# biomedia-mira/causal-gen

Hardware: AMD Instinct MI355X
Metric: HVAE train images/sec (higher is better)
Workload: dtype f16; 1 GPU; ukbb192 HVAE train step (192x192x1, DGauss likelihood, beta=5.0, z_max_res=96); per_gpu_batch=32, global_batch=32, parallelism=dp1, hipgraph=True, params=17371122

## Files before the change

causal-gen_amd/_lib.py:

```python
import ctypes as C
import os

_HERE = os.path.dirname(os.path.abspath(__file__))
LIB_PATH = os.environ.get("CGEN_LIB") or os.path.join(_HERE, "libcgen_hip.so")

F32, F16, F32S = 0, 1, 2
DMOL_LOW_BIT = 0x100
ACT_NONE, ACT_RELU, ACT_GELU = 0, 1, 2
UNARY_LEAKY_RELU, UNARY_CLAMP_MIN, UNARY_ADD = 3, 4, 5
MAX_SEG = 4


class View(C.Structure):
    _fields_ = [("p", C.c_void_p), ("sn", C.c_int64), ("sh", C.c_int64), ("sw", C.c_int64), ("c", C.c_int32),
                ("cpad", C.c_int32)]


NULL_VIEW = View(None, 0, 0, 0, 0, 0)


class ConvArgs(C.Structure):
    _fields_ = [("dtype", C.c_int32), ("n", C.c_int32), ("h", C.c_int32), ("w", C.c_int32), ("ks", C.c_int32),
                ("nseg", C.c_int32), ("act", C.c_int32), ("dact", C.c_int32), ("seg", View * MAX_SEG),
                ("weight", C.c_void_p), ("bias", C.c_void_p), ("out", View), ("aux", View), ("res1", View), ("res2", View),
                ("out_rem", C.c_int64), ("res1_rem", C.c_int64)]


class Block3Out(C.Structure):
    _fields_ = [("w", C.c_void_p), ("bias", C.c_void_p), ("out", View), ("aux", View), ("res1", View),
                ("out_rem", C.c_int64), ("res1_rem", C.c_int64)]


class Block3Args(C.Structure):
    _fields_ = [("dtype", C.c_int32), ("n", C.c_int32), ("h", C.c_int32), ("w", C.c_int32), ("nseg", C.c_int32),
                ("nout", C.c_int32), ("pre_act", C.c_int32), ("reserved", C.c_int32), ("seg", View * MAX_SEG),
                ("w_a", C.c_void_p), ("bias_a", C.c_void_p), ("mid", View), ("mid_aux", View), ("o", Block3Out * 2), ("w_a16", C.c_void_p)]


class Block4Args(C.Structure):
    _fields_ = [("dtype", C.c_int32), ("n", C.c_int32), ("h", C.c_int32), ("w", C.c_int32), ("nseg", C.c_int32),
                ("nout", C.c_int32), ("fwd", C.c_int32), ("b", C.c_int32), ("seg", View * MAX_SEG),
                ("wimg", C.c_void_p * 3), ("bias", C.c_void_p * 3), ("mid", View * 3), ("mid_aux", View * 3), ("o", Block3Out * 3)]


class WgradArgs(C.Structure):
    _fields_ = [("dtype", C.c_int32), ("n", C.c_int32), ("h", C.c_int32), ("w", C.c_int32), ("ks", C.c_int32),
                ("nseg", C.c_int32), ("act", C.c_int32), ("nsplit", C.c_int32), ("seg", View * MAX_SEG), ("gout", View),
                ("partial_w", C.c_void_p), ("partial_b", C.c_void_p)]


class WprepDesc(C.Structure):
    _fields_ = [("src", C.c_void_p), ("dst", C.c_void_p), ("co", C.c_int32), ("ci_total", C.c_int32), ("ks", C.c_int32),
                ("mode", C.c_int32), ("nseg", C.c_int32), ("seg_off", C.c_int32), ("seg_c", C.c_int32 * MAX_SEG),
                ("dtype", C.c_int32), ("rows_pad", C.c_int32), ("k_pad", C.c_int32), ("reserved", C.c_int32),
                ("numel", C.c_int64)]


class WredDesc(C.Structure):
    _fields_ = [("partial_w", C.c_void_p), ("partial_b", C.c_void_p), ("grad_w", C.c_void_p), ("grad_b", C.c_void_p),
                ("co", C.c_int32), ("ci_total", C.c_int32), ("ks", C.c_int32), ("nsplit", C.c_int32),
                ("accumulate", C.c_int32), ("unscale", C.c_float), ("layout", C.c_int32), ("reserved", C.c_int32),
                ("numel", C.c_int64)]


class AdamwArgs(C.Structure):
    _fields_ = [("p", C.c_void_p), ("g", C.c_void_p), ("m", C.c_void_p), ("v", C.c_void_p), ("ema", C.c_void_p),
                ("count", C.c_int64), ("lr", C.c_float), ("beta1", C.c_float), ("beta2", C.c_float), ("eps", C.c_float),
                ("wd", C.c_float), ("ema_beta", C.c_float), ("warmup_steps", C.c_int32), ("ema_update_after", C.c_int32),
                ("state_dev", C.c_void_p)]


class PredHead(C.Structure):
    _fields_ = [("c", C.c_int32), ("res", C.c_int32), ("width", C.c_int32), ("nout", C.c_int32), ("ctx", C.c_int32),
                ("kind", C.c_int32), ("tanh_loc", C.c_int32), ("obs_stride", C.c_int32), ("std_fixed", C.c_float),
                ("reserved", C.c_int32), ("w", C.c_void_p * 8), ("b", C.c_void_p * 8), ("y", C.c_void_p), ("obs", C.c_void_p)]


class PredTrainHead(C.Structure):
    _fields_ = [("hd", PredHead), ("gamma", C.c_void_p * 7), ("beta", C.c_void_p * 7), ("running_mean", C.c_void_p * 7),
                ("running_var", C.c_void_p * 7), ("num_batches_tracked", C.c_void_p * 7), ("gw", C.c_void_p * 8), ("gb", C.c_void_p),
                ("ggamma", C.c_void_p * 7), ("gbeta", C.c_void_p * 7)]


class AugmentArgs(C.Structure):
    _fields_ = [("dtype", C.c_int32), ("n", C.c_int32), ("c", C.c_int32), ("h0", C.c_int32), ("w0", C.c_int32), ("r_h", C.c_int32),
                ("r_w", C.c_int32), ("pad_x", C.c_int32), ("pad_y", C.c_int32), ("ctx", C.c_int32), ("stream_id", C.c_uint32),
                ("hflip_p", C.c_float), ("sub", C.c_float), ("mul", C.c_float), ("n_data", C.c_int64), ("data", C.c_void_p),
                ("index", C.c_void_p), ("out", View), ("rng", C.c_void_p), ("draws_in", C.c_void_p), ("draws_out", C.c_void_p),
                ("pa_data", C.c_void_p), ("pa_out", C.c_void_p)]


class LatentTailArgs(C.Structure):
    _fields_ = [("dtype", C.c_int32), ("n", C.c_int32), ("h", C.c_int32), ("w", C.c_int32), ("z_dim", C.c_int32), ("c", C.c_int32),
                ("coef_stride", C.c_int32), ("acc_q", C.c_int32), ("acc_p", C.c_int32), ("logt", C.c_float), ("parity", C.c_int32), ("reserved", C.c_int32),
                ("g_h", View), ("g_f", View), ("gz_in", View), ("q_loc", View), ("q_ls", View), ("p_loc", View), ("p_ls", View),
                ("z", View), ("out_p", View), ("out_q", View), ("img_fz", C.c_void_p), ("img_fp", C.c_void_p), ("img_pz", C.c_void_p),
                ("coef", C.c_void_p), ("chan_scale", C.c_void_p)]


class LatentTailFwdArgs(C.Structure):
    _fields_ = [("dtype", C.c_int32), ("n", C.c_int32), ("h", C.c_int32), ("w", C.c_int32), ("z_dim", C.c_int32), ("c", C.c_int32),
                ("ctx", C.c_int32), ("kl_stride", C.c_int32), ("stream_id", C.c_uint32), ("logt", C.c_float),
                ("h_in_rem", C.c_int64), ("h_out_rem", C.c_int64),
                ("q_loc", View), ("q_ls", View), ("p_loc", View), ("p_ls", View), ("p_feat", View), ("h_in", View), ("pa", View),
                ("eps", View), ("z", View), ("h_out", View), ("zf", View), ("img_p", C.c_void_p), ("img_f", C.c_void_p),
                ("bias_p", C.c_void_p), ("bias_f", C.c_void_p), ("rng", C.c_void_p), ("kl_part", C.c_void_p)]


class MetricVar(C.Structure):
    _fields_ = [("kind", C.c_int32), ("transform", C.c_int32), ("ncls", C.c_int32), ("reserved", C.c_int32), ("pred", C.c_void_p),
                ("pred_stride", C.c_int64), ("target", C.c_void_p), ("target_stride", C.c_int64), ("pred_scale", C.c_float),
                ("pred_shift", C.c_float), ("tgt_scale", C.c_float), ("tgt_shift", C.c_float), ("norm", C.c_float),
                ("reserved2", C.c_int32), ("acc", C.c_void_p), ("scores", C.c_void_p), ("labels", C.c_void_p),
                ("capacity", C.c_int64), ("row_count", C.c_void_p)]


class PgmMech(C.Structure):
    _fields_ = [("kind", C.c_int32), ("normalize", C.c_int32), ("col", C.c_int32), ("ncls", C.c_int32), ("nctx", C.c_int32),
                ("ctx_col", C.c_int32 * 2), ("nhidden", C.c_int32), ("width", C.c_int32 * 3), ("act", C.c_int32), ("bins", C.c_int32),
                ("bound", C.c_float), ("p", C.c_void_p * 8), ("g", C.c_void_p * 8)]


class PgmPre(C.Structure):
    _fields_ = [("col", C.c_int32), ("width", C.c_int32), ("kind", C.c_int32), ("hi", C.c_float), ("lo", C.c_float), ("mu", C.c_float),
                ("sd", C.c_float)]


class PgmCfArgs(C.Structure):
    _fields_ = [("obs", C.c_void_p), ("table_rows", C.c_int64), ("index", C.c_void_p), ("do_table", C.c_void_p), ("do_rows", C.c_int64),
                ("do_index", C.c_void_p), ("do_mask_dev", C.c_void_p), ("uniforms", C.c_void_p * 8), ("cf", C.c_void_p), ("eps", C.c_void_p),
                ("pa", C.c_void_p), ("cf_pa", C.c_void_p), ("ncol", C.c_int32), ("rows", C.c_int32), ("do_mask", C.c_uint32),
                ("exact_gumbel", C.c_int32), ("npre", C.c_int32), ("reserved", C.c_int32), ("pre", PgmPre * 8)]


PGM_BERNOULLI, PGM_CATEGORICAL, PGM_SPLINE, PGM_AFFINE, PGM_GUMBEL_MAX = 0, 1, 2, 3, 4
PGM_LEAKY_RELU, PGM_GELU, PGM_SIGMOID = 0, 1, 2
PGM_MAX_MECH, PGM_MAX_WIDTH, PGM_MAX_HIDDEN, PGM_MAX_BINS, PGM_MAX_CLS, PGM_ROWS = 8, 64, 3, 8, 16, 64
PGM_MAX_PRE, PGM_PRE_COPY, PGM_PRE_LOGSTD = 8, 0, 1
METRIC_BINARY, METRIC_CATEGORICAL, METRIC_CONTINUOUS = 0, 1, 2
METRIC_NONE, METRIC_SIGMOID, METRIC_SOFTMAX, METRIC_TANH = 0, 1, 2, 3
METRIC_N, METRIC_CORRECT, METRIC_ABS_ERR, METRIC_SKIPPED, METRIC_OVERFLOW = 0, 1, 2, 3, 4
METRIC_MAX_VARS, METRIC_ACC = 8, 8
STREAM_AUGMENT = 980
PRED_NORMAL, PRED_CATEGORICAL, PRED_BERNOULLI = 0, 1, 2
PRED_MAX_HEADS, PRED_MAX_OUT = 4, 16

i32, i64, u32, u64, f32, vp = C.c_int32, C.c_int64, C.c_uint32, C.c_uint64, C.c_float, C.c_void_p

PROTOTYPES = {
    "cgen_version": [],
    "cgen_h16_format": [],
    "cgen_last_error": [],
    "cgen_conv2d": [C.POINTER(ConvArgs), vp],
    "cgen_conv2d_pair_supported": [C.POINTER(ConvArgs), C.POINTER(ConvArgs)],
    "cgen_conv2d_pair": [C.POINTER(ConvArgs), C.POINTER(ConvArgs), vp],
    "cgen_block3_supported": [C.POINTER(Block3Args)],
    "cgen_block3": [C.POINTER(Block3Args), vp],
    "cgen_block3_pair_supported": [C.POINTER(Block3Args), C.POINTER(Block3Args)],
    "cgen_block3_pair": [C.POINTER(Block3Args), C.POINTER(Block3Args), vp],
    "cgen_block4_supported": [C.POINTER(Block4Args)],
    "cgen_block4": [C.POINTER(Block4Args), vp],
    "cgen_block4_pair_supported": [C.POINTER(Block4Args), C.POINTER(Block4Args)],
    "cgen_block4_pair": [C.POINTER(Block4Args), C.POINTER(Block4Args), vp],
    "cgen_conv2d_wgrad_plan": [C.POINTER(WgradArgs), C.POINTER(i32)],
    "cgen_conv2d_wgrad_batch_plan": [vp, i32, vp, i64, vp, vp, i32, vp, vp],
    "cgen_conv2d_wgrad_batch_run": [vp, vp, i32, i32, vp],
    "cgen_conv2d_wgrad": [C.POINTER(WgradArgs), vp],
    "cgen_weight_prep": [vp, vp, vp, i32, vp],
    "cgen_wgrad_reduce": [vp, vp, vp, i32, vp],
    "cgen_avgpool_fwd": [i32, i32, i32, i32, i32, View, View, vp],
    "cgen_avgpool_bwd": [i32, i32, i32, i32, i32, View, View, i32, vp],
    "cgen_adaptive_avgpool_fwd": [i32, i32, i32, i32, i32, i32, View, View, vp],
    "cgen_adaptive_avgpool_bwd": [i32, i32, i32, i32, i32, i32, View, View, i32, vp],
    "cgen_upsample_fwd": [i32, i32, i32, i32, i32, i32, View, vp, View, vp],
    "cgen_upsample_bwd": [i32, i32, i32, i32, i32, i32, View, View, i32, vp],
    "cgen_batch_reduce": [i32, i32, i32, i32, View, vp, i32, f32, vp],
    "cgen_batch_broadcast": [i32, i32, i32, i32, vp, View, vp],
    "cgen_axpby": [i32, i32, i32, i32, View, View, f32, f32, i32, i32, vp],
    "cgen_nchw_to_nhwc": [i32, i32, i32, i32, i32, i32, vp, View, f32, f32, vp],
    "cgen_nhwc_to_nchw": [i32, i32, i32, i32, i32, View, vp, vp],
    "cgen_batch_augment": [C.POINTER(AugmentArgs), vp],
    "cgen_batch_augment_arm": [C.POINTER(AugmentArgs)],
    "cgen_stem_conv_supported": [i32, i32, i32, i32],
    "cgen_stem_conv_fwd": [i32, i32, i32, i32, i32, i32, i32, View, vp, vp, View, vp],
    "cgen_im2col": [i32, i32, i32, i32, i32, View, View, vp],
    "cgen_reparam_kl_chunks": [i32, i32, i32],
    "cgen_reparam_kl_fwd": [i32, i32, i32, i32, i32, View, View, View, View, View, vp, u32, f32, View, View, vp, i32, vp],
    "cgen_reparam_kl_bwd": [i32, i32, i32, i32, i32, View, View, View, View, View, f32, View, vp, i32, vp, View, View, View,
                            View, i32, i32, vp],
    "cgen_reparam_kl_bwd_rider": [i32, i32, i32, i32, i32, View, View, View, View, View, f32, View, vp, i32, vp, View, View, View,
                                  View, i32, i32, View, View, i32, vp],
    "cgen_latent_tail_bwd_supported": [C.POINTER(LatentTailArgs)],
    "cgen_latent_tail_bwd": [C.POINTER(LatentTailArgs), vp],
    "cgen_latent_tail_fwd_supported": [C.POINTER(LatentTailFwdArgs)],
    "cgen_latent_tail_fwd": [C.POINTER(LatentTailFwdArgs), vp],
    "cgen_kl_channel_sums": [i32, i32, i32, i32, i32, View, View, View, View, f32, vp, i32, vp],
    "cgen_elbo_finalize_fb": [i32, vp, i32, f32, vp, i32, f32, f32, f32, vp, vp, vp, vp],
    "cgen_im2col_strided": [i32, i32, i32, i32, i32, i32, i32, i32, i32, View, View, vp],
    "cgen_col2im_strided": [i32, i32, i32, i32, i32, i32, i32, i32, i32, View, View, i32, vp],
    "cgen_unary_fwd": [i32, i32, f32, i32, i32, i32, i32, View, View, vp],
    "cgen_unary_bwd": [i32, i32, f32, i32, i32, i32, i32, View, View, View, i32, vp],
    "cgen_sample_gaussian": [i32, i32, i32, i32, i32, View, View, View, vp, u32, f32, View, vp],
    "cgen_gaussian_kl_map": [i64, vp, vp, vp, vp, vp, vp],
    "cgen_mediator_mix": [i32, i32, i32, i32, i32, View, View, View, View, View, f32, f32, f32, i32, View, vp],
    "cgen_like_chunks": [i32, i32],
    "cgen_dgauss_nll_fwd": [i32, i32, i32, i32, i32, View, View, vp, vp],
    "cgen_dgauss_nll_bwd": [i32, i32, i32, i32, i32, View, View, vp, i32, View, vp],
    "cgen_dgauss_params": [i32, i32, i32, i32, i32, View, View, f32, vp, vp, vp],
    "cgen_dgauss_sample": [i32, i32, i32, i32, i32, View, f32, vp, u32, vp, vp, vp],
    "cgen_gauss_nll_fwd": [i32, i32, i32, i32, i32, View, View, View, vp, u32, vp, vp],
    "cgen_gauss_nll_bwd": [i32, i32, i32, i32, i32, View, View, View, vp, u32, vp, i32, View, vp],
    "cgen_gauss_sample": [i32, i32, i32, i32, i32, View, f32, vp, u32, vp, vp, vp],
    "cgen_dmol_nll_fwd": [i32, i32, i32, i32, View, View, vp, vp],
    "cgen_dmol_nll_bwd": [i32, i32, i32, i32, View, View, vp, i32, View, vp],
    "cgen_dmol_decode": [i32, i32, i32, i32, View, i32, vp, u32, f32, vp, vp, vp],
    "cgen_dmol_decode_bwd": [i32, i32, i32, i32, View, i32, vp, u32, f32, vp, vp, f32, View, vp],
    "cgen_elbo_finalize": [i32, vp, i32, f32, vp, i32, f32, f32, vp, vp, vp],
    "cgen_cf_dgauss_bwd": [i32, i32, i32, i32, i32, View, View, View, vp, f32, View, View, vp],
    "cgen_cf_dmol_bwd": [i32, i32, i32, i32, i32, View, View, View, vp, f32, View, View, vp],
    "cgen_cf_pixels": [i64, vp, vp, vp, vp, vp, vp, vp, vp, vp],
    "cgen_sumsq_partial": [vp, i64, vp, i32, vp],
    "cgen_clip_decide": [vp, i32, vp, f32, f32, vp, vp],
    "cgen_adamw_ema": [C.POINTER(AdamwArgs), vp],
    "cgen_step_commit": [vp, vp],
    "cgen_predictor_supported": [C.POINTER(PredHead), i32],
    "cgen_predictor_workspace": [C.POINTER(PredHead), i32, C.POINTER(i64)],
    "cgen_predictor_fwd": [C.POINTER(PredHead), i32, i32, vp, vp, vp, vp, vp, vp],
    "cgen_predictor_bwd": [C.POINTER(PredHead), i32, i32, vp, vp, vp, vp, vp],
    "cgen_predictor_tiled_supported": [C.POINTER(PredHead), i32],
    "cgen_predictor_tiled_workspace": [C.POINTER(PredHead), i32, i32, C.POINTER(i64)],
    "cgen_predictor_tiled_fwd": [C.POINTER(PredHead), i32, i32, vp, vp, i64, vp, vp, vp, vp],
    "cgen_predictor_tiled_bwd": [C.POINTER(PredHead), i32, i32, vp, vp, i64, vp, vp, vp],
    "cgen_predictor_train_workspace": [C.POINTER(PredTrainHead), i32, i32, C.POINTER(i64)],
    "cgen_predictor_train_fwd": [C.POINTER(PredTrainHead), i32, i32, vp, vp, i64, f32, vp, vp, vp, vp],
    "cgen_predictor_train_bwd": [C.POINTER(PredTrainHead), i32, i32, vp, vp, i64, vp, vp, vp],
    "cgen_pgm_workspace": [C.POINTER(PgmMech), i32, i32, C.POINTER(i64)],
    "cgen_pgm_nll_fwd": [C.POINTER(PgmMech), i32, vp, i32, i64, vp, i32, vp, vp, vp],
    "cgen_pgm_nll_fwd_bwd": [C.POINTER(PgmMech), i32, vp, i32, i64, vp, i32, vp, vp, vp, vp, i64, vp],
    "cgen_pgm_counterfactual": [C.POINTER(PgmMech), i32, C.POINTER(PgmCfArgs), vp],
    "cgen_metric_accum": [C.POINTER(MetricVar), i32, i32, vp],
    "cgen_rocauc": [vp, vp, vp, i64, i32, i64, vp, vp, vp],
    "cgen_image_dist": [i32, i64, vp, vp, vp, vp, vp, vp],
    "cgen_philox_normal": [vp, i64, vp, u32, vp],
    "cgen_rng_advance": [vp, u64, vp],
}
_RESTYPES = {"cgen_last_error": C.c_char_p}
ABI_VERSION = 411
_NOCHECK = {"cgen_version", "cgen_h16_format", "cgen_last_error", "cgen_conv2d_wgrad_plan", "cgen_reparam_kl_chunks", "cgen_like_chunks",
            "cgen_block3_supported", "cgen_block4_supported", "cgen_block4_pair_supported", "cgen_block3_pair_supported", "cgen_conv2d_pair_supported", "cgen_stem_conv_supported",
            "cgen_predictor_supported", "cgen_predictor_tiled_supported", "cgen_batch_augment_arm", "cgen_latent_tail_bwd_supported", "cgen_latent_tail_fwd_supported"}


# ... 56 lines not shown
```

causal-gen_amd/csrc/conv.hip:

```cpp
#include <stdlib.h>

#include <algorithm>
#include <type_traits>
#include <vector>

#include "common.h"
#include "wgrad3.h"

#ifdef CGEN_NO_SETPRIO
#define CGEN_SETPRIO() do {} while (0)
#else
#define CGEN_SETPRIO() __builtin_amdgcn_s_setprio(3)
#endif

namespace cgen {

typedef float f32x4 __attribute__((ext_vector_type(4)));
typedef unsigned int u32x4 __attribute__((ext_vector_type(4)));

struct FastDiv {
  uint32_t mul, shift, d, pad;
};
static inline FastDiv mk_fastdiv(uint32_t d) {
  FastDiv f;
// ... 2850 lines not shown
    }
  }
  return check_launch("cgen_conv2d_wgrad_batch_run");
}

extern "C" int cgen_conv2d_wgrad(const cgen_wgrad_args* a, cgen_stream_t stream) {
  CGEN_REQUIRE(a && a->partial_w, "cgen_conv2d_wgrad: null args");
  CGEN_REQUIRE(a->dtype == CGEN_F32 || a->dtype == CGEN_F16, "cgen_conv2d_wgrad: bad dtype");
  CGEN_REQUIRE(a->nseg >= 1 && a->nseg <= CGEN_MAX_SEG && a->gout.p && a->gout.c > 0, "cgen_conv2d_wgrad: bad args");
  const int esz = a->dtype == CGEN_F32 ? 4 : 2;
  WgP p;
  memset(&p, 0, sizeof(p));
  p.N = a->n; p.H = a->h; p.W = a->w; p.KS = a->ks; p.pad = a->ks / 2; p.nseg = a->nseg; p.act = a->act;
  p.Co = a->gout.c; p.P = a->n * a->h * a->w; p.taps = a->ks * a->ks;
  int off = 0, ch = 0;
  for (int s = 0; s < a->nseg; ++s) {
    p.seg[s] = mk(a->seg[s]);
    p.seg_off[s] = off;
    p.seg_vec[s] = vec16_ok(a->seg[s], esz);
    p.seg_chunk0[s] = ch;
    off += a->seg[s].c;
    ch += (a->seg[s].c + 31) / 32;
  }
  p.seg_chunk0[a->nseg] = ch;
  p.ci_total = off;
  p.n_cichunks = ch;
  p.n_tapgroups = ceil_div(p.taps, WG_MAXT);
  {
    Wg3Plan g3;
    if (wg3_plan(a, g3)) {
      CGEN_REQUIRE(g3.nsplit_total == a->nsplit, "cgen_conv2d_wgrad: nsplit %d != expected %d", a->nsplit, g3.nsplit_total);
      wg3_launch_single(g3, (hipStream_t)stream);
      return check_launch("cgen_conv2d_wgrad(stream)");
    }
  }
  {
    int segc[CGEN_MAX_SEG];
    for (int s = 0; s < a->nseg; ++s) segc[s] = a->seg[s].c;
    Wg2Geom g;
    Wg2P q;
    if (build_wg2(a, q, g)) {
      CGEN_REQUIRE(g.nsplit == a->nsplit, "cgen_conv2d_wgrad: nsplit %d != expected %d", a->nsplit, g.nsplit);
      { const char* e = getenv("CGEN_WG2_DBG"); q.dbg = e ? atoi(e) : 0; }
      { const char* e = getenv("CGEN_WG2_STAMPS"); q.stamps = e ? (unsigned long long*)strtoull(e, nullptr, 0) : nullptr; }
      hipStream_t st = (hipStream_t)stream;
      switch (g.ncf) {
        case 1: launch_wgrad2_ks<1, 16>(q, g, st); break;
        case 2: if (a->ks == 7 || g.njw == 16) launch_wgrad2_ks<2, 16>(q, g, st); else launch_wgrad2_ks<2, 12>(q, g, st); break;
        case 4: launch_wgrad2_ks<4, 6>(q, g, st); break;
        case 6: launch_wgrad2_ks<6, 4>(q, g, st); break;
        default: launch_wgrad2_ks<8, 3>(q, g, st); break;
      }
      return check_launch("cgen_conv2d_wgrad(tile)");
    }
  }
  int ns, pps;
  wgrad_geometry(p.P, p.Co, (p.ci_total + 31) / 32, p.KS, ns, pps);
  CGEN_REQUIRE(ns == a->nsplit, "cgen_conv2d_wgrad: nsplit %d != expected %d", a->nsplit, ns);
  p.nsplit = ns; p.pix_per_split = pps;
  p.gout = mk(a->gout);
  {
    const int q = 4 * esz;
    p.gout_vec = ((uintptr_t)a->gout.p % q == 0) && ((a->gout.sn * esz) % q == 0) && ((a->gout.sh * esz) % q == 0) && ((a->gout.sw * esz) % q == 0);
  }
  p.pw = a->partial_w; p.pb = a->partial_b;
  return a->dtype == CGEN_F32 ? launch_wgrad<float>(p, (hipStream_t)stream) : launch_wgrad<h16_t>(p, (hipStream_t)stream);
}

extern "C" int cgen_weight_prep(const cgen_wprep_desc* descs, const int32_t* csite, const int32_t* cidx, int32_t nchunks,
                                cgen_stream_t stream) {
  if (nchunks <= 0) return CGEN_OK;
  CGEN_REQUIRE(descs && csite && cidx, "cgen_weight_prep: null table");
  hipLaunchKernelGGL(wprep_kernel, dim3(nchunks), dim3(256), 0, (hipStream_t)stream, descs, csite, cidx);
  return check_launch("cgen_weight_prep");
}

extern "C" int cgen_wgrad_reduce(const cgen_wred_desc* descs, const int32_t* csite, const int32_t* cidx, int32_t nchunks,
                                 cgen_stream_t stream) {
  if (nchunks <= 0) return CGEN_OK;
  CGEN_REQUIRE(descs && csite && cidx, "cgen_wgrad_reduce: null table");
  hipLaunchKernelGGL(wred_kernel, dim3(nchunks), dim3(256), 0, (hipStream_t)stream, descs, csite, cidx);
  return check_launch("cgen_wgrad_reduce");
}
```

causal-gen_amd/wgrad_sched.py:

```python
import ctypes as C
import os

import torch

from . import _lib


class WgradMixin:
    @staticmethod
    def _needs_wgrad(site):
        b = site.conv.bias
        return site.conv.weight.requires_grad or (b is not None and b.requires_grad)

    def _wgrad(self, site, segs, act, g):
        x0 = segs[0]
        a = _lib.WgradArgs()
        gn, gh, gw, vw = self._geom(site.ks, list(segs) + [g])
        a.dtype, a.n, a.h, a.w, a.ks, a.nseg, a.act = self.dt, gn, gh, gw, site.ks, len(segs), act
        for k, s in enumerate(segs):
            a.seg[k] = vw(s)
        a.gout = vw(g)
        use = sum(1 for e in self._wg_events if e[0] is site)
        lay = tuple((v.sn, v.sh, v.sw, v.c, v.p % 16 if v.p else 0) for v in [a.seg[k] for k in range(len(segs))] + [a.gout])
        key = (site.index, use, x0.n, x0.h, x0.w, lay)
        ent = self._partials.get(key)
        nw = site.co * site.taps * site.ci
        if ent is None:
            kind = C.c_int32(0)
            nsplit = self.lib.conv2d_wgrad_plan(C.byref(a), C.byref(kind))
            ent = (torch.empty(nsplit * (nw + site.co), dtype=torch.float32, device=self.device), nsplit, 1 if kind.value == 3 else 0)
            self._partials[key] = ent
        buf, nsplit, _layout = ent
        a.nsplit = nsplit
        a.partial_w = buf.data_ptr()
        a.partial_b = buf.data_ptr() + 4 * nsplit * nw if site.conv.bias is not None else None
        if self._defer_wgrad():
            cost = 2.0 * site.ci * site.taps * site.co * x0.n * x0.h * x0.w
            self._wg_deferred.append((a, cost))
            self._wg_cum += cost
            self._wgrad_marks()
        else:
            self._timed("conv_wgrad", [site], x0, lambda: self.lib.conv2d_wgrad(C.byref(a), self.stream))
        self._wg_events.append((site, key, nsplit))

    def _wgrad_marks(self):
        k = self._wg_nflush
        if self._in_side:
            return
        if (self.wgrad_batch and self.prof is None and k < len(self.wgrad_flush_frac) and self._wg_total > 0
                and self._wg_cum >= self.wgrad_flush_frac[k] * self._wg_total):
            self._wg_nflush += 1
            self._launch_batched_wgrads(background=True)
        if (self.on_split is not None and not self._split_done and self._wg_nflush >= max(1, len(self.wgrad_flush_frac)) and self._wg_total > 0
                and self._wg_cum >= self.split_frac * self._wg_total):
            self._split_done = True
            if self._wg_forked:
                main = torch.cuda.current_stream(self.device)
                for st in self._wg_pool:
                    main.wait_stream(st)
                self._wg_forked = False
            final = set()
            for st_, _, _ in self._wg_events[:self._wg_reduced]:
                final.add(id(st_.conv.weight))
                if st_.conv.bias is not None:
                    final.add(id(st_.conv.bias))
            self.early_final = final
            self.on_split()

    def _launch_deferred_wgrads(self, final=True):
        main = torch.cuda.current_stream(self.device)
        if self.wgrad_batch:
            if self._wg_deferred:
                self._launch_batched_wgrads()
            if final and self._wg_forked:
                for st in self._wg_pool:
                    main.wait_stream(st)
                self._wg_forked = False
            return
        if self._wg_deferred:
            k = min(self.wgrad_streams, len(self._wg_deferred))
            while len(self._wg_pool) < k:
                self._wg_pool.append(torch.cuda.Stream(self.device))
            streams = self._wg_pool[:k]
            for st in streams:
                st.wait_stream(main)
            self._wg_forked = True
            load = [0.0] * k
            for a, cost in sorted(self._wg_deferred, key=lambda e: -e[1]):
# ... 76 lines not shown
                for k, (c0, c1) in enumerate(zip(snap, self.arena.chunks)):
                    d = (c0 != c1).nonzero().flatten()
                    print("straycheck chunk %d: %d arena bytes changed by the flushed batch (arena offset now %d of chunk %d)%s" % (
                        k, d.numel(), self.arena.off, self.arena.ci, "" if not d.numel() else " first %d last %d" % (int(d[0]), int(d[-1]))), flush=True)
            return
        if blob is not None and nl:
            self.lib.conv2d_wgrad_batch_run(blob.data_ptr(), launches, nl, 0, self.stream)
            self.launches += nl
        if len(rest) >= 4 and self.wgrad_streams > 1 and ev is None:
            main = torch.cuda.current_stream(self.device)
            k = min(self.wgrad_streams, len(rest))
            while len(self._wg_pool) < k:
                self._wg_pool.append(torch.cuda.Stream(self.device))
            costs = [c for _, c in self._wg_deferred]
            load = [0.0] * k
            for st in self._wg_pool[:k]:
                st.wait_stream(main)
            for i in sorted(rest, key=lambda i: -costs[i]):
                j = load.index(min(load))
                load[j] += costs[i] + 2.0e8
                self.lib.conv2d_wgrad(C.byref(args[i]), self._wg_pool[j].cuda_stream)
                self.launches += 1
            for st in self._wg_pool[:k]:
                main.wait_stream(st)
        else:
            for i in rest:
                self.lib.conv2d_wgrad(C.byref(args[i]), self.stream)
                self.launches += 1
        if ev is not None:
            ev[1].record()
            ent2 = self.prof.setdefault(("conv_wgrad", 0, 0, 0, 0), [0.0, [], 0])
            ent2[0] += sum(c for _, c in self._wg_deferred)
            ent2[1].append(ev)
            ent2[2] += nl + len(rest)
        self._wg_deferred = []

    def _reduce_wgrads(self):
        self._launch_deferred_wgrads()
        self._reduce_events(self.stream)

    def _reduce_events(self, stream):
        events = self._wg_events[self._wg_reduced:]
        if not events:
            return
        self._wg_reduced = len(self._wg_events)
        rounds, nth = [], {}
        for ev in events:
            k = nth.get(ev[0].index, 0)
            nth[ev[0].index] = k + 1
            while len(rounds) <= k:
                rounds.append([])
            rounds[k].append(ev)
        for evs in rounds:
            self._reduce_round(evs, stream)

    def _reduce_round(self, events, stream):
        flags = []
        for site, _, _ in events:
            flags.append(site.index in self._wg_seen)
            self._wg_seen.add(site.index)
        sig = (tuple(k for _, k, _ in events), tuple(flags), self.loss_scale)
        tab = self._red_tabs.get(sig)
        if tab is None:
            descs, csite, cidx = [], [], []
            for (site, key, nsplit), acc in zip(events, flags):
                buf = self._partials[key][0]
                nw = site.co * site.taps * site.ci
                d = _lib.WredDesc()
                d.partial_w = buf.data_ptr()
                d.partial_b = buf.data_ptr() + 4 * nsplit * nw if site.conv.bias is not None else None
                d.grad_w = self.param_grad_ptr(site.conv.weight)
                d.grad_b = self.param_grad_ptr(site.conv.bias) if site.conv.bias is not None else None
                d.co, d.ci_total, d.ks, d.nsplit = site.co, site.ci, site.ks, nsplit
                d.layout = self._partials[key][2]
                d.accumulate = 1 if acc else 0
                d.unscale = 1.0 / self.loss_scale
                d.numel = nw + (site.co if site.conv.bias is not None else 0)
                descs.append(d)
            for i, d in enumerate(descs):
                nch = (d.numel + self.CHUNK - 1) // self.CHUNK
                csite += [i] * nch
                cidx += list(range(nch))
            arr = (_lib.WredDesc * len(descs))(*descs)
            tab = (self._to_dev(bytes(arr)), torch.tensor(csite, dtype=torch.int32, device=self.device),
                   torch.tensor(cidx, dtype=torch.int32, device=self.device), len(csite))
            self._red_tabs[sig] = tab
        d, cs, ci, n = tab
        self.lib.wgrad_reduce(d.data_ptr(), cs.data_ptr(), ci.data_ptr(), n, stream)
        self.launches += 1
        for site, _, _ in events:
            if site.conv.weight.requires_grad:
                self.pgrad_init.add(id(site.conv.weight))
            if site.conv.bias is not None and site.conv.bias.requires_grad:
                self.pgrad_init.add(id(site.conv.bias))
```

include/cgen_hip.h:

```cpp
#ifndef CGEN_HIP_H
#define CGEN_HIP_H

#include <stddef.h>
#include <stdint.h>

#ifdef __cplusplus
extern "C" {
#endif

typedef void* cgen_stream_t;

enum cgen_status { CGEN_OK = 0, CGEN_EINVAL = -1, CGEN_ELAUNCH = -2, CGEN_EUNSUPPORTED = -3 };
enum cgen_dtype { CGEN_F32 = 0, CGEN_F16 = 1,
                  CGEN_F32S = 2 };
enum cgen_act { CGEN_ACT_NONE = 0, CGEN_ACT_RELU = 1, CGEN_ACT_GELU = 2 };

typedef struct cgen_view {
  void* p;
  int64_t sn, sh, sw;
  int32_t c;
  int32_t cpad;
} cgen_view;

#define CGEN_MAX_SEG 4
// ... 13 lines not shown
  int64_t out_rem, res1_rem;
} cgen_conv_args;
int cgen_conv2d(const cgen_conv_args* a, cgen_stream_t stream);
int cgen_conv2d_pair_supported(const cgen_conv_args* a, const cgen_conv_args* b);
int cgen_conv2d_pair(const cgen_conv_args* a, const cgen_conv_args* b, cgen_stream_t stream);

typedef struct cgen_block3_out {
  const void* w;
  const float* bias;
  cgen_view out, aux, res1;
  int64_t out_rem, res1_rem;
} cgen_block3_out;
typedef struct cgen_block3_args {
  int32_t dtype, n, h, w, nseg, nout, pre_act, reserved;
  cgen_view seg[CGEN_MAX_SEG];
  const void* w_a;
  const float* bias_a;
  cgen_view mid, mid_aux;
  cgen_block3_out o[2];
  const void* w_a16;
} cgen_block3_args;
int cgen_block3_supported(const cgen_block3_args* a);
int cgen_block3(const cgen_block3_args* a, cgen_stream_t stream);
int cgen_block3_pair_supported(const cgen_block3_args* a, const cgen_block3_args* b);
int cgen_block3_pair(const cgen_block3_args* a, const cgen_block3_args* b, cgen_stream_t stream);

typedef struct cgen_block4_args {
  int32_t dtype, n, h, w, nseg, nout, fwd, b;
  cgen_view seg[CGEN_MAX_SEG];
  const void* wimg[3];
  const float* bias[3];
  cgen_view mid[3], mid_aux[3];
  cgen_block3_out o[3];
} cgen_block4_args;
int cgen_block4_supported(const cgen_block4_args* a);
int cgen_block4(const cgen_block4_args* a, cgen_stream_t stream);
int cgen_block4_pair_supported(const cgen_block4_args* a, const cgen_block4_args* b);
int cgen_block4_pair(const cgen_block4_args* a, const cgen_block4_args* b, cgen_stream_t stream);

typedef struct cgen_wgrad_args {
  int32_t dtype, n, h, w, ks, nseg, act, nsplit;
  cgen_view seg[CGEN_MAX_SEG];
  cgen_view gout;
  float* partial_w;
  float* partial_b;
} cgen_wgrad_args;
int cgen_conv2d_wgrad_plan(const cgen_wgrad_args* a, int32_t* tiled_out);
typedef struct {
  int32_t ncf, ks, lds_bytes, nblocks;
  int64_t blocks_offset;
} cgen_wgrad_batch_launch;
int cgen_conv2d_wgrad_batch_plan(const cgen_wgrad_args* args, int32_t count, void* blob_host, int64_t capacity, int64_t* blob_bytes,
                                 cgen_wgrad_batch_launch* launches, int32_t max_launches, int32_t* n_launches, int32_t* eligible);
int cgen_conv2d_wgrad_batch_run(const void* blob_dev, const cgen_wgrad_batch_launch* launches, int32_t n_launches, int32_t max_workgroups,
                               cgen_stream_t);
int cgen_conv2d_wgrad(const cgen_wgrad_args* a, cgen_stream_t stream);

typedef struct cgen_wprep_desc {
  const float* src;
  void* dst;
  int32_t co, ci_total, ks, mode;
  int32_t nseg, seg_off;
  int32_t seg_c[CGEN_MAX_SEG];
  int32_t dtype, rows_pad, k_pad, reserved;
  int64_t numel;
} cgen_wprep_desc;
int cgen_weight_prep(const cgen_wprep_desc* descs_dev, const int32_t* chunk_site_dev, const int32_t* chunk_index_dev,
                     int32_t nchunks, cgen_stream_t stream);

typedef struct cgen_wred_desc {
  const float* partial_w;
  const float* partial_b;
  float* grad_w;
  float* grad_b;
  int32_t co, ci_total, ks, nsplit;
  int32_t accumulate;
  float unscale;
  int32_t layout;
  int32_t reserved;
  int64_t numel;
} cgen_wred_desc;
int cgen_wgrad_reduce(const cgen_wred_desc* descs_dev, const int32_t* chunk_site_dev, const int32_t* chunk_index_dev,
                      int32_t nchunks, cgen_stream_t stream);

int cgen_avgpool_fwd(int32_t dtype, int32_t n, int32_t ho, int32_t wo, int32_t d, cgen_view in, cgen_view out, cgen_stream_t);
int cgen_avgpool_bwd(int32_t dtype, int32_t n, int32_t ho, int32_t wo, int32_t d, cgen_view gout, cgen_view gin,
                     int32_t accumulate, cgen_stream_t);
int cgen_adaptive_avgpool_fwd(int32_t dtype, int32_t n, int32_t hi, int32_t wi, int32_t ho, int32_t wo, cgen_view in, cgen_view out,
                              cgen_stream_t);
int cgen_adaptive_avgpool_bwd(int32_t dtype, int32_t n, int32_t hi, int32_t wi, int32_t ho, int32_t wo, cgen_view gout, cgen_view gin,
                              int32_t accumulate, cgen_stream_t);
int cgen_upsample_fwd(int32_t dtype, int32_t n, int32_t hi, int32_t wi, int32_t ho, int32_t wo, cgen_view in,
                      const float* bias, cgen_view out, cgen_stream_t);
int cgen_upsample_bwd(int32_t dtype, int32_t n, int32_t hi, int32_t wi, int32_t ho, int32_t wo, cgen_view gout,
                      cgen_view gin, int32_t accumulate, cgen_stream_t);
int cgen_batch_reduce(int32_t dtype, int32_t n, int32_t h, int32_t w, cgen_view in, float* out, int32_t accumulate,
                      float unscale, cgen_stream_t);
int cgen_batch_broadcast(int32_t dtype, int32_t n, int32_t h, int32_t w, const float* src, cgen_view out, cgen_stream_t);
int cgen_axpby(int32_t dtype, int32_t n, int32_t h, int32_t w, cgen_view in, cgen_view out, float alpha, float beta,
               int32_t c_from, int32_t accumulate, cgen_stream_t);
int cgen_nchw_to_nhwc(int32_t src_is_u8, int32_t dtype, int32_t n, int32_t c, int32_t h, int32_t w, const void* src,
                      cgen_view out, float sub, float mul, cgen_stream_t);
int cgen_stem_conv_supported(int32_t dtype, int32_t cin, int32_t ks, int32_t co);
int cgen_stem_conv_fwd(int32_t dtype, int32_t n, int32_t h, int32_t w, int32_t cin, int32_t ks, int32_t co, cgen_view in,
                       const float* weight_oihw, const float* bias, cgen_view out, cgen_stream_t);
int cgen_im2col(int32_t dtype, int32_t n, int32_t h, int32_t w, int32_t ks, cgen_view in, cgen_view out, cgen_stream_t);
int cgen_im2col_strided(int32_t dtype, int32_t n, int32_t h, int32_t w, int32_t ks, int32_t stride, int32_t pad, int32_t ho,
                        int32_t wo, cgen_view in, cgen_view out, cgen_stream_t);
int cgen_col2im_strided(int32_t dtype, int32_t n, int32_t h, int32_t w, int32_t ks, int32_t stride, int32_t pad, int32_t ho,
                        int32_t wo, cgen_view gcol, cgen_view gin, int32_t accumulate, cgen_stream_t);
#define CGEN_UNARY_LEAKY_RELU 3
#define CGEN_UNARY_CLAMP_MIN 4
#define CGEN_UNARY_ADD 5
int cgen_unary_fwd(int32_t dtype, int32_t op, float param, int32_t n, int32_t h, int32_t w, int32_t c, cgen_view in, cgen_view out,
                   cgen_stream_t);
int cgen_unary_bwd(int32_t dtype, int32_t op, float param, int32_t n, int32_t h, int32_t w, int32_t c, cgen_view x, cgen_view gout,
                   cgen_view gin, int32_t accumulate, cgen_stream_t);
int cgen_nhwc_to_nchw(int32_t dtype, int32_t n, int32_t c, int32_t h, int32_t w, cgen_view in, float* dst, cgen_stream_t);

typedef struct cgen_augment_args {
  int32_t dtype;
  int32_t n, c, h0, w0;
  int32_t r_h, r_w;
  int32_t pad_x, pad_y;
  int32_t ctx;
  uint32_t stream_id;
  float hflip_p, sub, mul;
  int64_t n_data;
  const void* data;
  const int64_t* index;
  cgen_view out;
  const uint64_t* rng;
  const int32_t* draws_in;
  int32_t* draws_out;
  const float* pa_data;
  float* pa_out;
} cgen_augment_args;
int cgen_batch_augment(const cgen_augment_args* a, cgen_stream_t stream);
int cgen_batch_augment_arm(const cgen_augment_args* a);

int cgen_reparam_kl_chunks(int32_t h, int32_t w, int32_t c);
int cgen_reparam_kl_fwd(int32_t dtype, int32_t n, int32_t h, int32_t w, int32_t c, cgen_view q_loc, cgen_view q_ls,
                        cgen_view p_loc, cgen_view p_ls, cgen_view eps_in, const uint64_t* rng, uint32_t stream_id,
                        float logt, cgen_view z, cgen_view eps_out, float* kl_part, int32_t kl_stride, cgen_stream_t);
int cgen_reparam_kl_bwd(int32_t dtype, int32_t n, int32_t h, int32_t w, int32_t c, cgen_view q_loc, cgen_view q_ls,
                        cgen_view p_loc, cgen_view p_ls, cgen_view z, float logt, cgen_view gz,
                        const float* kl_coef_dev, int32_t coef_stride, const float* kl_chan_scale, cgen_view g_q_loc,
                        cgen_view g_q_ls, cgen_view g_p_loc, cgen_view g_p_ls, int32_t acc_q, int32_t acc_p, cgen_stream_t);
int cgen_reparam_kl_bwd_rider(int32_t dtype, int32_t n, int32_t h, int32_t w, int32_t c, cgen_view q_loc, cgen_view q_ls,
                              cgen_view p_loc, cgen_view p_ls, cgen_view z, float logt, cgen_view gz,
                              const float* kl_coef_dev, int32_t coef_stride, const float* kl_chan_scale, cgen_view g_q_loc,
                              cgen_view g_q_ls, cgen_view g_p_loc, cgen_view g_p_ls, int32_t acc_q, int32_t acc_p,
                              cgen_view ride_src, cgen_view ride_dst, int32_t ride_acc, cgen_stream_t);
int cgen_kl_channel_sums(int32_t dtype, int32_t n, int32_t h, int32_t w, int32_t c, cgen_view q_loc, cgen_view q_ls,
                         cgen_view p_loc, cgen_view p_ls, float logt, float* out, int32_t out_stride, cgen_stream_t);
int cgen_gaussian_kl_map(int64_t count, const float* q_loc, const float* q_ls, const float* p_loc, const float* p_ls,
                         float* out, cgen_stream_t);
int cgen_sample_gaussian(int32_t dtype, int32_t n, int32_t h, int32_t w, int32_t c, cgen_view loc, cgen_view ls,
                         cgen_view eps_in, const uint64_t* rng, uint32_t stream_id, float logt, cgen_view z,
                         cgen_stream_t);
int cgen_mediator_mix(int32_t dtype, int32_t n, int32_t h, int32_t w, int32_t c, cgen_view z, cgen_view q_loc,
                      cgen_view q_ls, cgen_view p_loc, cgen_view p_ls, float alpha, float t, float logt, int32_t linear_var, cgen_view out,
                      cgen_stream_t);

typedef struct cgen_latent_tail_bwd_args {
  int32_t dtype, n, h, w, z_dim, c;
// ... 236 lines not shown
```

Measured before the change: 2424 images/s.

## Replace wgrad split-reduction with a tiled multi-tensor reduce kernel

Adds a new tiled kernel that reduces split-K weight-gradient partials. Each block handles a host-planned tile of output rows and columns, sums across splits with vectorized nontemporal loads, stages the sums in shared memory, and writes them out in the target layout (including the flipped-tap transpose layout). Items are sorted so that long split chains are scheduled first. The intent is better coalescing and load balance than the per-chunk reduce kernel, at the cost of host-side planning complexity and a larger device-side item table. The old path stays reachable through an environment variable.

```diff
diff --git a/causal-gen_amd/_lib.py b/causal-gen_amd/_lib.py
--- a/causal-gen_amd/_lib.py
+++ b/causal-gen_amd/_lib.py
@@ -61,6 +61,13 @@
                 ("co", C.c_int32), ("ci_total", C.c_int32), ("ks", C.c_int32), ("nsplit", C.c_int32),
                 ("accumulate", C.c_int32), ("unscale", C.c_float), ("layout", C.c_int32), ("reserved", C.c_int32),
                 ("numel", C.c_int64)]
+
+
+class WredItem(C.Structure):
+    _fields_ = [("partial", C.c_void_p), ("grad", C.c_void_p), ("kind", C.c_int32), ("nsplit", C.c_int32),
+                ("split_stride", C.c_int32), ("vec", C.c_int32), ("v4", C.c_int32), ("accumulate", C.c_int32),
+                ("unscale", C.c_float), ("taps", C.c_int32), ("inner", C.c_int32), ("ci_total", C.c_int32), ("layout", C.c_int32),
+                ("a0", C.c_int32), ("na", C.c_int32), ("b0", C.c_int32), ("nb", C.c_int32), ("reserved", C.c_int32)]
 
 
 class AdamwArgs(C.Structure):
@@ -168,6 +175,9 @@
     "cgen_conv2d_wgrad": [C.POINTER(WgradArgs), vp],
     "cgen_weight_prep": [vp, vp, vp, i32, vp],
     "cgen_wgrad_reduce": [vp, vp, vp, i32, vp],
+    "cgen_weight_prep_ref": [vp, vp, vp, i32, vp],
+    "cgen_wgrad_reduce_tiles": [vp, i32, vp],
+    "cgen_wgrad_reduce_ref": [vp, vp, vp, i32, vp],
     "cgen_avgpool_fwd": [i32, i32, i32, i32, i32, View, View, vp],
     "cgen_avgpool_bwd": [i32, i32, i32, i32, i32, View, View, i32, vp],
     "cgen_adaptive_avgpool_fwd": [i32, i32, i32, i32, i32, i32, View, View, vp],
diff --git a/causal-gen_amd/csrc/conv.hip b/causal-gen_amd/csrc/conv.hip
--- a/causal-gen_amd/csrc/conv.hip
+++ b/causal-gen_amd/csrc/conv.hip
@@ -2956,3 +2956,13 @@
   hipLaunchKernelGGL(wred_kernel, dim3(nchunks), dim3(256), 0, (hipStream_t)stream, descs, csite, cidx);
   return check_launch("cgen_wgrad_reduce");
 }
+
+extern "C" int cgen_weight_prep_ref(const cgen_wprep_desc* descs, const int32_t* csite, const int32_t* cidx, int32_t nchunks,
+                                    cgen_stream_t stream) {
+  return cgen_weight_prep(descs, csite, cidx, nchunks, stream);
+}
+
+extern "C" int cgen_wgrad_reduce_ref(const cgen_wred_desc* descs, const int32_t* csite, const int32_t* cidx, int32_t nchunks,
+                                     cgen_stream_t stream) {
+  return cgen_wgrad_reduce(descs, csite, cidx, nchunks, stream);
+}
diff --git a/causal-gen_amd/csrc/multitensor.hip b/causal-gen_amd/csrc/multitensor.hip
--- /dev/null
+++ b/causal-gen_amd/csrc/multitensor.hip
@@ -0,0 +1,159 @@
+#include "common.h"
+
+namespace cgen {
+
+#define WRED_T 2048
+#define WRED_T_DEEP 1024
+
+template <int VW>
+__device__ __forceinline__ void wred_load(const float* q, float* t) {
+  if (VW == 4) { const f32x4_t v = __builtin_nontemporal_load((const f32x4_t*)q); t[0] = v[0]; t[1 % VW] = v[1]; t[2 % VW] = v[2]; t[3 % VW] = v[3]; }
+  else t[0] = __builtin_nontemporal_load(q);
+}
+
+template <int VW>
+__device__ __forceinline__ void wred_chain(const float* p, size_t stride, int c, int step, int nsplit, float* out) {
+  float acc[VW];
+#pragma unroll
+  for (int e = 0; e < VW; ++e) acc[e] = 0.f;
+  int sp = c;
+  for (; sp + 7 * step < nsplit; sp += 8 * step) {
+    float t[8][VW];
+#pragma unroll
+    for (int j = 0; j < 8; ++j) {
+      wred_load<VW>(p + (size_t)(sp + j * step) * stride, t[j]);
+    }
+#pragma unroll
+    for (int j = 0; j < 8; ++j)
+#pragma unroll
+      for (int e = 0; e < VW; ++e) acc[e] += t[j][e];
+  }
+  for (; sp < nsplit; sp += step) {
+    float v[VW];
+    wred_load<VW>(p + (size_t)sp * stride, v);
+#pragma unroll
+    for (int e = 0; e < VW; ++e) acc[e] += v[e];
+  }
+#pragma unroll
+  for (int e = 0; e < VW; ++e) out[e] = acc[e];
+}
+
+template <int VW>
+__device__ __forceinline__ void wred_tile_sums(const cgen_wred_item& it, float* sm, int n, bool deep) {
+  const int ngroups = n / VW;
+  const size_t stride = (size_t)it.split_stride;
+  const float* base = it.partial + ((size_t)it.a0 * it.taps * it.inner + it.b0);
+  if (it.nsplit <= 4) {
+    for (int u0 = threadIdx.x; u0 < ngroups; u0 += 2 * 256) {
+      float t[2][4][VW];
+#pragma unroll
+      for (int j = 0; j < 2; ++j) {
+        const int l = (u0 + 256 * j) * VW;
+        if (l < n) {
+          const int row = (int)((unsigned)l / (unsigned)it.nb), col = l - row * it.nb;
+          const float* q = base + (size_t)row * it.inner + col;
+#pragma unroll
+          for (int c = 0; c < 4; ++c)
+            if (c < it.nsplit) wred_load<VW>(q + (size_t)c * stride, t[j][c]);
+        }
+      }
+#pragma unroll
+      for (int j = 0; j < 2; ++j) {
+        const int l = (u0 + 256 * j) * VW;
+        if (l < n) {
+#pragma unroll
+          for (int e = 0; e < VW; ++e) {
+            float r;
+            if (it.vec) {
+              float b[4];
+#pragma unroll
+              for (int c = 0; c < 4; ++c) { b[c] = 0.f; if (c < it.nsplit) b[c] += t[j][c][e]; }
+              r = (b[0] + b[1]) + (b[2] + b[3]);
+            } else {
+              r = 0.f;
+#pragma unroll
+              for (int c = 0; c < 4; ++c) if (c < it.nsplit) r += t[j][c][e];
+            }
+            sm[l + e] = r;
+          }
+        }
+      }
+    }
+    return;
+  }
+  if (!deep) {
+    for (int u = threadIdx.x; u < ngroups; u += 256) {
+      const int l = u * VW, row = (int)((unsigned)l / (unsigned)it.nb), col = l - row * it.nb;
+      float a[VW];
+      wred_chain<VW>(base + (size_t)row * it.inner + col, stride, 0, 1, it.nsplit, a);
+#pragma unroll
+      for (int e = 0; e < VW; ++e) sm[l + e] = a[e];
+    }
+    return;
+  }
+  const int units = 4 * ngroups;
+  for (int u = threadIdx.x; u < units; u += 256) {
+    const int c = (int)((unsigned)u / (unsigned)ngroups), l = (u - c * ngroups) * VW;
+    const int row = (int)((unsigned)l / (unsigned)it.nb), col = l - row * it.nb;
+    float a[VW];
+    wred_chain<VW>(base + (size_t)row * it.inner + col, stride, c, 4, it.nsplit, a);
+#pragma unroll
+    for (int e = 0; e < VW; ++e) sm[c * n + l + e] = a[e];
+  }
+}
+
+__global__ __launch_bounds__(256) void wred_kernel_tiled(const cgen_wred_item* items) {
+  __shared__ float sm[4 * WRED_T_DEEP];
+  const cgen_wred_item it = items[blockIdx.x];
+  const float us = it.unscale == 0.f ? 1.f : it.unscale;
+  if (it.kind == 1) {
+    for (int e = threadIdx.x; e < it.nb; e += 256) {
+      const float* p = it.partial + it.b0 + e;
+      float acc = 0.f;
+      int sp = 0;
+      for (; sp + 16 <= it.nsplit; sp += 16) {
+        float t[16];
+#pragma unroll
+        for (int c = 0; c < 16; ++c) t[c] = p[(size_t)(sp + c) * it.split_stride];
+#pragma unroll
+        for (int c = 0; c < 16; ++c) acc += t[c];
+      }
+      for (; sp < it.nsplit; ++sp) acc += p[(size_t)sp * it.split_stride];
+      float* g = it.grad + it.b0 + e;
+      *g = it.accumulate ? *g + acc * us : acc * us;
+    }
+    return;
+  }
+  const bool deep = it.vec && it.nsplit > 4;
+  const int n = it.na * it.taps * it.nb;
+  if (n <= 0 || n > (deep ? WRED_T_DEEP : WRED_T) || it.nb <= 0 || it.taps <= 0 || (it.v4 && (it.nb & 3))) return;
+  if (it.v4) wred_tile_sums<4>(it, sm, n, deep); else wred_tile_sums<1>(it, sm, n, deep);
+  __syncthreads();
+  const int run = (it.layout == 1 ? it.na : it.nb) * it.taps;
+  for (int m = threadIdx.x; m < n; m += 256) {
+    const int q = (int)((unsigned)m / (unsigned)run), r = m - q * run;
+    const int x = (int)((unsigned)r / (unsigned)it.taps), tt = r - x * it.taps;
+    int l;
+    size_t o;
+    if (it.layout == 1) {
+      l = (x * it.taps + (it.taps - 1 - tt)) * it.nb + q;
+      o = ((size_t)(it.b0 + q) * it.ci_total + it.a0) * it.taps + r;
+    } else {
+      l = (q * it.taps + tt) * it.nb + x;
+      o = ((size_t)(it.a0 + q) * it.ci_total + it.b0) * it.taps + r;
+    }
+    const float s = deep ? (sm[l] + sm[n + l]) + (sm[2 * n + l] + sm[3 * n + l]) : sm[l];
+    it.grad[o] = it.accumulate ? it.grad[o] + s * us : s * us;
+  }
+}
+
+}
+
+using namespace cgen;
+
+extern "C" int cgen_wgrad_reduce_tiles(const cgen_wred_item* items, int32_t nitems, cgen_stream_t stream) {
+  if (nitems <= 0) return CGEN_OK;
+  CGEN_REQUIRE(items, "cgen_wgrad_reduce_tiles: null table");
+  hipLaunchKernelGGL(wred_kernel_tiled, dim3(nitems), dim3(256), 0, (hipStream_t)stream, items);
+  return check_launch("cgen_wgrad_reduce_tiles");
+}
diff --git a/causal-gen_amd/wgrad_sched.py b/causal-gen_amd/wgrad_sched.py
--- a/causal-gen_amd/wgrad_sched.py
+++ b/causal-gen_amd/wgrad_sched.py
@@ -4,6 +4,57 @@
 import torch
 
 from . import _lib
+
+
+WRED_TILE, WRED_TILE_DEEP = 2048, 1024
+_WRED_REF = os.environ.get("CGEN_WRED_REF", "0") == "1"
+
+
+def _even_cut(n, most):
+    if n <= most:
+        return n
+    most = max(most - most % 4, 1) if most >= 4 else most
+    cuts = -(-n // most)
+    w = -(-n // cuts)
+    return min(most, -(-w // 4) * 4 if most >= 4 else w)
+
+
+def plan_wred_items(descs):
+    items = []
+    for d in descs:
+        taps, co, ci = d.ks * d.ks, d.co, d.ci_total
+        nw = co * ci * taps
+        assert taps <= WRED_TILE and nw < 2 ** 31
+        pw = d.partial_w or 0
+        vec = 1 if nw % 4 == 0 and pw % 16 == 0 else 0
+        tile = WRED_TILE_DEEP if vec and d.nsplit > 4 else WRED_TILE
+        if d.layout == 1:
+            rows, inner = ci, co
+            na = min(rows, max(1, -(-64 // taps)))
+            nb = _even_cut(inner, max(1, tile // (na * taps)))
+            na = min(rows, max(1, tile // (taps * nb)))
+        else:
+            rows, inner = co, ci
+            nb = _even_cut(inner, max(1, tile // taps))
+            na = min(rows, max(1, tile // (taps * nb)))
+        for a0 in range(0, rows, na):
+            for b0 in range(0, inner, nb):
+                it = _lib.WredItem()
+                it.partial, it.grad, it.kind, it.nsplit, it.split_stride = d.partial_w, d.grad_w, 0, d.nsplit, nw
+                it.vec, it.accumulate, it.unscale = vec, d.accumulate, d.unscale
+                it.taps, it.inner, it.ci_total, it.layout = taps, inner, ci, d.layout
+                it.a0, it.na, it.b0, it.nb = a0, min(na, rows - a0), b0, min(nb, inner - b0)
+                it.v4 = 1 if vec and inner % 4 == 0 and it.b0 % 4 == 0 and it.nb % 4 == 0 else 0
+                assert 0 < it.na * taps * it.nb <= tile
+                items.append(it)
+        if d.grad_b:
+            for b0 in range(0, co, 1024):
+                it = _lib.WredItem()
+                it.partial, it.grad, it.kind, it.nsplit, it.split_stride = d.partial_b, d.grad_b, 1, d.nsplit, co
+                it.accumulate, it.unscale, it.b0, it.nb = d.accumulate, d.unscale, b0, min(1024, co - b0)
+                items.append(it)
+    items.sort(key=lambda it: -(it.nsplit if it.kind == 1 or not it.vec else (it.nsplit + 3) // 4))
+    return (_lib.WredItem * len(items))(*items)
 
 
 class WgradMixin:
@@ -246,11 +297,16 @@
                 csite += [i] * nch
                 cidx += list(range(nch))
             arr = (_lib.WredDesc * len(descs))(*descs)
+            items = plan_wred_items(descs)
             tab = (self._to_dev(bytes(arr)), torch.tensor(csite, dtype=torch.int32, device=self.device),
-                   torch.tensor(cidx, dtype=torch.int32, device=self.device), len(csite))
+                   torch.tensor(cidx, dtype=torch.int32, device=self.device), len(csite),
+                   self._to_dev(bytes(items)), len(items))
             self._red_tabs[sig] = tab
-        d, cs, ci, n = tab
-        self.lib.wgrad_reduce(d.data_ptr(), cs.data_ptr(), ci.data_ptr(), n, stream)
+        d, cs, ci, n, items, nitems = tab
+        if _WRED_REF:
+            self.lib.wgrad_reduce_ref(d.data_ptr(), cs.data_ptr(), ci.data_ptr(), n, stream)
+        else:
+            self.lib.wgrad_reduce_tiles(items.data_ptr(), nitems, stream)
         self.launches += 1
         for site, _, _ in events:
             if site.conv.weight.requires_grad:
diff --git a/include/cgen_hip.h b/include/cgen_hip.h
--- a/include/cgen_hip.h
+++ b/include/cgen_hip.h
@@ -119,6 +119,26 @@
 } cgen_wred_desc;
 int cgen_wgrad_reduce(const cgen_wred_desc* descs_dev, const int32_t* chunk_site_dev, const int32_t* chunk_index_dev,
                       int32_t nchunks, cgen_stream_t stream);
+
+int cgen_weight_prep_ref(const cgen_wprep_desc* descs_dev, const int32_t* chunk_site_dev, const int32_t* chunk_index_dev,
+                         int32_t nchunks, cgen_stream_t stream);
+
+typedef struct cgen_wred_item {
+  const float* partial;
+  float* grad;
+  int32_t kind, nsplit;
+  int32_t split_stride;
+  int32_t vec;
+  int32_t v4;
+  int32_t accumulate;
+  float unscale;
+  int32_t taps, inner, ci_total, layout;
+  int32_t a0, na, b0, nb;
+  int32_t reserved;
+} cgen_wred_item;
+int cgen_wgrad_reduce_tiles(const cgen_wred_item* items_dev, int32_t nitems, cgen_stream_t stream);
+int cgen_wgrad_reduce_ref(const cgen_wred_desc* descs_dev, const int32_t* chunk_site_dev, const int32_t* chunk_index_dev,
+                          int32_t nchunks, cgen_stream_t stream);
 
 int cgen_avgpool_fwd(int32_t dtype, int32_t n, int32_t ho, int32_t wo, int32_t d, cgen_view in, cgen_view out, cgen_stream_t);
 int cgen_avgpool_bwd(int32_t dtype, int32_t n, int32_t ho, int32_t wo, int32_t d, cgen_view gout, cgen_view gin,
```

Result: faster. 2454 images/s (median of 6 runs) (+1.3%).
